# pglira/simpleICP

Measured on AMD Instinct MI355X. Metric: ICP iterations/sec (kNN correspondences/sec in `correspondences_per_s`), 10M-vs-10M pts, higher is better.
Workload: dtype f64; 1 GPU; C4 synthetic 10000000-vs-10000000 surface (SURVEY 8d generator), correspondences=1000, neighbors=10, exact 1-NN (bit-identical to brute force); n_fixed=10000000, n_movable=10000000, correspondences=1000, neighbors=10, parallelism=movable-cloud index shards x1, queries replicated

## Files before the change

### simpleicp_amd/csrc/sicp_api.cpp

```cpp
#include "sicp_host.h"
#include "../../include/simpleicp_hip_chain.h"

namespace sicph {

thread_local std::string g_err;

int fail(int code, const char *fmt, ...)
{
    char buf[512];
    va_list ap;
    va_start(ap, fmt);
    vsnprintf(buf, sizeof buf, fmt, ap);
    va_end(ap);
    g_err = buf;
    return code;
}

}

int sicp_io_fail(int code, const char *fmt, ...)
{
    char buf[512];
    va_list ap;
    va_start(ap, fmt);
// ... 154 lines not shown
    if (!ctx_out) return fail(SICP_ERR_INVALID, "ctx_out is null");
    *ctx_out = nullptr;
    int n = 0;
    if (hipGetDeviceCount(&n) != hipSuccess || n <= 0)
        return fail(SICP_ERR_NO_DEVICE, "no HIP device visible: libsimpleicp_hip has no CPU path");
    if (device < 0 || device >= n) return fail(SICP_ERR_INVALID, "device %d out of range [0,%d)", device, n);
    HIPCHK(hipSetDevice(device));
    sicp_ctx *c = new sicp_ctx();
    c->device = device;
    if (hipGetDeviceProperties(&c->prop, device) != hipSuccess) { delete c; return fail(SICP_ERR_HIP, "hipGetDeviceProperties failed"); }
    if (std::strncmp(c->prop.gcnArchName, "gfx950", 6) != 0) {
        const std::string arch = c->prop.gcnArchName;
        delete c;
        return fail(SICP_ERR_NO_DEVICE, "device %d is %s; this library carries gfx950 code only", device, arch.c_str());
    }
    if (hipStreamCreateWithFlags(&c->stream, hipStreamNonBlocking) != hipSuccess) { delete c; return fail(SICP_ERR_HIP, "hipStreamCreate failed"); }
    if (hipHostMalloc((void **)&c->h_small, H_SMALL_WORDS * sizeof(double), hipHostMallocMapped) != hipSuccess) { delete c; return fail(SICP_ERR_HIP, "hipHostMalloc failed"); }
    int rc = c->small.reserve(128);
    if (rc == SICP_OK) rc = c->ne_partial.reserve((size_t)NE_MAX_GRID * 64);
    if (rc == SICP_OK) rc = c->ticket.reserve(4);
    if (rc == SICP_OK) rc = c->icp_dev.reserve(1);
    if (rc == SICP_OK && hipStreamCreateWithFlags(&c->stream2, hipStreamNonBlocking) != hipSuccess) rc = SICP_ERR_HIP;
    if (rc == SICP_OK && hipEventCreateWithFlags(&c->pre_ev, hipEventDisableTiming) != hipSuccess) rc = SICP_ERR_HIP;
    if (rc == SICP_OK) rc = c->pre_tkt.reserve(PRE_TKT_WORDS);
    if (rc == SICP_OK && hipMemsetAsync(c->pre_tkt.p, 0, PRE_TKT_WORDS * sizeof(unsigned long long), c->stream) != hipSuccess) rc = SICP_ERR_HIP;
    if (rc == SICP_OK) rc = c->lm_dev.reserve(1);
    if (rc == SICP_OK && hipHostMalloc((void **)&c->h_lm, sizeof(LmDev), hipHostMallocDefault) != hipSuccess) rc = SICP_ERR_HIP;
    if (rc == SICP_OK) rc = c->match_work.reserve(8);
    if (rc == SICP_OK && hipMemsetAsync(c->match_work.p, 0, 8 * sizeof(unsigned long long), c->stream) != hipSuccess) rc = SICP_ERR_HIP;
    if (rc == SICP_OK && hipHostMalloc((void **)&c->h_rec, (size_t)REC_RING * REC_DOUBLES * sizeof(double), hipHostMallocMapped) != hipSuccess) rc = SICP_ERR_HIP;
    if (rc == SICP_OK && hipHostMalloc((void **)&c->h_state, sizeof(IcpDev), hipHostMallocDefault) != hipSuccess) rc = SICP_ERR_HIP;
    if (rc == SICP_OK) std::memset(c->h_rec, 0, (size_t)REC_RING * REC_DOUBLES * sizeof(double));
    if (rc == SICP_OK && hipMemsetAsync(c->ticket.p, 0, 4 * sizeof(unsigned), c->stream) != hipSuccess) rc = SICP_ERR_HIP;
    if (rc != SICP_OK) { sicp_ctx_destroy(c); return rc; }
    if (const char *e = std::getenv("SICP_ORDER_MIN_Q")) c->order_min_q = std::atol(e);
    if (const char *e = std::getenv("SICP_KNN_SWEEP")) c->knn_sweep = std::atoi(e) != 0;
    if (const char *e = std::getenv("SICP_KNN_BATCH")) c->knn_batch = std::atol(e);
    if (const char *e = std::getenv("SICP_KNN_GROUP")) c->knn_group = std::atoi(e);
    if (const char *e = std::getenv("SICP_NN16_MIN_Q")) c->nn16_min_q = std::atol(e);
    if (const char *e = std::getenv("SICP_NN16")) c->nn16_filter = !std::strcmp(e, "exact") ? 0 : !std::strcmp(e, "far") ? 1 : 2;
    if (const char *e = std::getenv("SICP_BOXES")) { c->use_boxes = std::atoi(e) != 0; c->boxes_always = std::atoi(e) >= 2; }
    if (const char *e = std::getenv("SICP_NN16F_MIN_Q")) { c->nn16f_min_q = std::atol(e); c->nn16f_min_q_forced = true; }
    if (const char *e = std::getenv("SICP_FAR_MOVE")) { const double t = std::atof(e); if (t >= 0) c->far_move = t; }
    if (const char *e = std::getenv("SICP_COARSE_MIN_N")) c->coarse_min_n = std::atol(e);
    if (const char *e = std::getenv("SICP_LM")) c->lm_one_launch = std::strcmp(e, "launches") != 0;
    if (const char *e = std::getenv("SICP_HSEL_WINDOW")) c->hsel_window = std::atoi(e) != 0;
    if (const char *e = std::getenv("SICP_TAIL_WINDOW")) c->tail_window = std::atoi(e) != 0;
    if (const char *e = std::getenv("SICP_CHAIN_PRELAUNCH")) c->chain_prelaunch = std::atoi(e) != 0;
    if (const char *e = std::getenv("SICP_TEST_BARRIER_FAULT")) c->test_barrier_fault = std::atoi(e);
    if (const char *e = std::getenv("SICP_NN_GROUP")) { const int v = std::atoi(e); if (v == 8 || v == 16) c->nn_group = v; }
    if (const char *e = std::getenv("SICP_XCHG_KEYS_MIN_Q")) c->xkeys_min_q = std::atol(e);
    if (const char *e = std::getenv("SICP_COMM_TIMEOUT_S")) { const double v = std::atof(e); if (v > 0) c->xchg_timeout_s = 2.0 * v; }
    if (const char *e = std::getenv("SICP_FSCAN")) c->fscan_variant = !std::strcmp(e, "inline") ? 1 : 0;
    if (const char *e = std::getenv("SICP_FSCAN_CAP")) c->fscan_cap = std::atol(e);
    if (const char *e = std::getenv("SICP_OUTLIER_CHUNK")) c->outlier_chunk = std::atol(e);
    if (const char *e = std::getenv("SICP_CLUSTER_CHUNK")) c->cluster_chunk = std::atol(e) > 0 ? std::atol(e) : (1L << 22);
    if (const char *e = std::getenv("SICP_FPFH_CHUNK")) c->fpfh_chunk = std::atol(e);
    if (const char *e = std::getenv("SICP_KEYPOINT_CHUNK")) c->keypoint_chunk = std::atol(e);
    if (const char *e = std::getenv("SICP_MATCH_CHUNK")) c->match_chunk = std::atol(e);
    if (const char *e = std::getenv("SICP_PLANE_SPAN")) c->plane_span = std::atol(e) > 0 ? std::atol(e) : 0;
    if (const char *e = std::getenv("SICP_ROBUST")) c->robust_path = !std::strcmp(e, "sweeps") ? 1 : !std::strcmp(e, "one") ? 2 : 0;
    if (const char *e = std::getenv("SICP_CONSISTENCY")) c->consistency_path = !std::strcmp(e, "sweeps") ? 1 : !std::strcmp(e, "one") ? 2 : 0;
    if (const char *e = std::getenv("SICP_SOLVE_TRACE")) {
        c->solve_trace = true;
        c->host_trace = std::strstr(e, "host") != nullptr;
        c->trace_sel = std::strstr(e, "sel") != nullptr; c->trace_eval = std::strstr(e, "eval") != nullptr;
    }
    if (const char *e = std::getenv("SICP_SOLVE")) c->solve_mode = !std::strcmp(e, "fused") ? 1 : !std::strcmp(e, "host") ? 2 : 0;
    if (const char *e = std::getenv("SICP_KNN1"))
        c->knn1_mode = !std::strcmp(e, "exact") ? 1 : !std::strcmp(e, "filter") ? 2 : !std::strcmp(e, "grid") ? 3 : 0;
    *ctx_out = c;
    return SICP_OK;
}

SICP_EXPORT int sicp_ctx_destroy(sicp_ctx *c)
{
    if (!c) return SICP_OK;
    (void)hipSetDevice(c->device);
    for (int s = 0; s < 2; ++s) (void)upload_join(c, s);
    if (c->copy_stream) { (void)hipStreamSynchronize(c->copy_stream); (void)hipStreamDestroy(c->copy_stream); c->copy_stream = nullptr; }
    if (c->h_bg) { (void)hipHostFree(c->h_bg); c->h_bg = nullptr; }
    c->stage_bg.release(); c->bg_small.release();
    if (c->stream) (void)hipStreamSynchronize(c->stream);
    if (c->stream2) { (void)hipStreamSynchronize(c->stream2); (void)hipStreamDestroy(c->stream2); c->stream2 = nullptr; }
    if (c->pre_ev) { (void)hipEventDestroy(c->pre_ev); c->pre_ev = nullptr; }
    c->pre_tkt.release();
    if (c->comm) { (void)rccl()->CommDestroy(c->comm); c->comm = nullptr; }
    if (c->h_dl && !c->dl_shared) (void)hipHostFree(c->h_dl);
    c->h_dl = nullptr;
    for (auto &e : c->dl_ev) if (e) { (void)hipEventDestroy(e); e = nullptr; }
    for (auto &p : c->pending) { (void)hipEventDestroy(p.a); (void)hipEventDestroy(p.b); }
    for (auto &p : c->pool) { (void)hipEventDestroy(p.a); (void)hipEventDestroy(p.b); }
    for (auto &cl : c->cloud) { cl.xyz.release(); cl.pl.release(); cl.grid.cell_start.release(); cl.grid.rec.release();
                                 cl.sub_xyz.release(); cl.sub_grid.cell_start.release(); cl.sub_grid.rec.release(); }
    c->bound_p2.release(); c->bound_d2.release(); c->bound_idx.release(); c->q_order.release(); c->k_order.release(); c->k_sel.release(); c->k_nv.release(); c->k_pl.release(); c->k_cov.release(); c->k_redo.release(); c->g_ids.release(); c->g_counts.release(); c->g_cursor.release(); c->g_blk.release(); c->match_work.release(); c->rj_keys.release();
    c->stage.release(); c->part_d2.release(); c->part_idx.release(); c->kq.release(); c->k_d2.release();
    c->k_idx.release(); c->floor_d2.release(); c->floor_idx.release(); c->bound.release(); c->hit_cnt.release(); c->hit_list.release(); c->x_send.release(); c->x_recv.release(); c->q.release(); c->normals.release();
    c->planarity.release(); c->m_idx.release(); c->m_d2.release(); c->m_p2.release(); c->dist.release();
    c->resid.release(); c->flag.release(); c->keep.release(); c->small.release(); c->ne_partial.release();
    c->lm_bar_buf.release(); c->lm_gsum.release(); c->ticket.release(); c->icp_dev.release(); c->lm_dev.release(); c->resid2.release();
    c->corr_pl.release();
    for (auto &cl : c->cloud) { cl.nv.release(); cl.nrm2.release(); cl.nrm2_have.release(); }
    c->na.cnt.release(); c->na.list_q.release(); c->na.list_m.release(); c->na.iota.release(); c->na.cov.release(); c->na.per_q.release();
    c->batch_tab.release(); c->batch_map.release();
    c->sel_blk.release(); c->sel_pos.release();
    c->vx_tab.release(); c->vx_slot.release(); c->cand_rows.release(); c->cand_keep.release(); c->cand_small.release();
    c->ev_part.release(); c->ev_out.release(); c->ev_cnt.release();
    c->ol_d.release(); c->ol_part.release(); c->ol_cnt.release();
// ... 115 lines not shown
```

### simpleicp_amd/csrc/sicp_handover.h

```cpp
#ifndef SICP_HANDOVER_H
#define SICP_HANDOVER_H

#include <cstdint>

namespace sicph {

constexpr int HANDOVER_RING = 16;

struct HandOverStep {
    int stream = 0;
    bool wait = false;
    unsigned long long wait_seq = 0;
    bool first_on_second = false;
    int slot = 0;
};

struct HandOver {
    bool road = false;
    int64_t launched = 0;
    int64_t early = 0;
    double last_seq = 0.0;
    bool second_used = false;

    HandOverStep next(double seq)
    {
        HandOverStep s;
        s.slot = (int)(launched % HANDOVER_RING);
        if (road) {
            s.stream = (int)(launched & 1);
            s.wait = launched > 0;
            s.wait_seq = s.wait ? (unsigned long long)last_seq : 0ull;
            s.first_on_second = s.stream == 1 && !second_used;
            if (s.stream == 1) second_used = true;
            if (s.wait) ++early;
        }
        last_seq = seq;
        ++launched;
        return s;
    }
};

}

#endif
```

### simpleicp_amd/csrc/sicp_host.h

```cpp
#ifndef SICP_HOST_H
#define SICP_HOST_H

#include <hip/hip_runtime.h>
#include <rccl/rccl.h>
#include <dlfcn.h>
#include <sched.h>

#include <algorithm>
#include <atomic>
#include <chrono>
#include <cmath>
#include <cstdarg>
#include <cstdio>
#include <cstdlib>
#include <cstring>
#include <limits>
#include <condition_variable>
#include <memory>
#include <mutex>
#include <string>
#include <thread>
#include <vector>

#include "../../include/simpleicp_hip.h"
// ... 86 lines not shown
    decltype(&ncclAllReduce) AllReduce = nullptr;
    decltype(&ncclGetErrorString) GetErrorString = nullptr;
    decltype(&ncclCommCount) CommCount = nullptr;
    decltype(&ncclCommUserRank) CommUserRank = nullptr;
    decltype(&ncclCommAbort) CommAbort = nullptr;
    std::string why;
};

struct NormalAngle {
    double cos_max = 0.0;
    int k = 0;
    int par = 0;
    long iota_n = 0;
    bool counters_stale = false;
    DevBuf<unsigned> cnt;
    DevBuf<uint32_t> list_q, list_m, iota;
    DevBuf<double> cov;
    DevBuf<float> per_q;
};

struct EventPair { hipEvent_t a, b; int kernel; };
constexpr int REC_RING = 16;
static_assert(REC_RING == HANDOVER_RING, "sicp_handover.h indexes the same ring");

inline long round_up(long v, long g) { return (v + g - 1) / g * g; }
inline double wall_ms() { return std::chrono::duration<double, std::milli>(std::chrono::steady_clock::now().time_since_epoch()).count(); }
inline bool is_observed(double w) { return w > 0 && std::isfinite(w); }
inline void H16_to_Xf(const double H[16], Xf *o) { for (int i = 0; i < 12; ++i) o->m[i] = H[i]; }

}
using namespace sicph;

struct BgUpload {
    std::thread th;
    bool active = false;
    int rc = SICP_OK;
    std::string err;
};

struct sicp_ctx {
    int device = 0;
    hipStream_t stream = nullptr;
    hipStream_t copy_stream = nullptr;
    BgUpload bg[2];
    DevBuf<double> stage_bg;
    DevBuf<double> bg_small;
// ... 85 lines not shown
    bool trace_sel = false, trace_eval = false;
    long solve_seq = 0;
    DevBuf<IcpDev> icp_dev;
    DevBuf<LmDev> lm_dev;
    LmDev *h_lm = nullptr;
    DevBuf<double> resid2;
    int resid_slot = 0;
    int lm_evals = 4;
    double *h_rec = nullptr;
    IcpDev *h_state = nullptr;
    DevBuf<unsigned long long> lm_bar_buf;
    unsigned long long lm_bar = 0;
    bool lm_one_launch = true;
    unsigned long long hsel_bar = 0;
    int test_barrier_fault = 0;
    bool tail_window = true;
    bool reject_prior = false;
    bool hsel_window = true;
    long hsel_run_launches = 0;
    bool hsel_dirty = false;
    int nn_group = 0;
    hipStream_t stream2 = nullptr;
    hipEvent_t pre_ev = nullptr;
    DevBuf<unsigned long long> pre_tkt;
    bool chain_prelaunch = true;
    bool pre_running = false;
    int64_t pre_last_run = 0, pre_total = 0;
    int chain_depth = 4;
    DevBuf<BatchMember> batch_tab;
    DevBuf<uint32_t> batch_map;
    double *h_batch_ring = nullptr;
    long batch_ring_members = 0;
    hipEvent_t batch_ev = nullptr;
    DevBuf<uint32_t> sel_blk;
    DevBuf<int64_t> sel_pos;
    DevBuf<int64_t> cand_rows;
    DevBuf<uint8_t> cand_keep;
    DevBuf<unsigned long long> cand_small;
    DevBuf<unsigned long long> vx_tab;
    DevBuf<uint32_t> vx_slot;
    DevBuf<double> ev_part, ev_out;
    DevBuf<long long> ev_cnt;
    DevBuf<double> ol_d, ol_part;
    DevBuf<uint32_t> ol_cnt;
    long outlier_chunk = 0;
    DevBuf<float> fp_nrm, fp_out;
    DevBuf<uint16_t> fp_cnt;
// ... 340 lines not shown
```

### simpleicp_amd/csrc/sicp_icp.cpp

```cpp
#include "sicp_host.h"
#include <map>

namespace sicph {

void euler_R(const double a[3], double R[9])
{
    const double c1 = std::cos(a[0]), s1 = std::sin(a[0]);
    const double c2 = std::cos(a[1]), s2 = std::sin(a[1]);
    const double c3 = std::cos(a[2]), s3 = std::sin(a[2]);
    R[0] = c2 * c3;                 R[1] = -c2 * s3;                R[2] = s2;
    R[3] = c1 * s3 + s1 * s2 * c3;  R[4] = c1 * c3 - s1 * s2 * s3;  R[5] = -s1 * c2;
    R[6] = s1 * s3 - c1 * s2 * c3;  R[7] = s1 * c3 + c1 * s2 * s3;  R[8] = c1 * c2;
}

void euler_dR(const double a[3], double dR[27])
{
    const double c1 = std::cos(a[0]), s1 = std::sin(a[0]);
    const double c2 = std::cos(a[1]), s2 = std::sin(a[1]);
    const double c3 = std::cos(a[2]), s3 = std::sin(a[2]);
    double *A = dR, *B = dR + 9, *C = dR + 18;
    A[0] = 0; A[1] = 0; A[2] = 0;
    A[3] = -s1 * s3 + c1 * s2 * c3;  A[4] = -s1 * c3 - c1 * s2 * s3;  A[5] = -c1 * c2;
    A[6] = c1 * s3 + s1 * s2 * c3;   A[7] = c1 * c3 - s1 * s2 * s3;   A[8] = -s1 * c2;
    B[0] = -s2 * c3;       B[1] = s2 * s3;        B[2] = c2;
// ... 171 lines not shown
    if (c->Q <= 0) return fail(SICP_ERR_INVALID, "call sicp_icp_setup first");
    CHK(check_slot(c, SICP_MOV, true));
    for (int j = 0; j < 6; ++j)
        if (std::isnan(P->obs_weight[j]) || P->obs_weight[j] < 0) return fail(SICP_ERR_INVALID, "obs_weight[%d] must be >= 0", j);
    return SICP_OK;
}

bool device_tail(const sicp_ctx *c) { return c->solve_mode != 2; }

int loop_state_init(sicp_ctx *c, const sicp_iter_params *P0)
{
    IcpDev &hs = *c->h_state;
    std::memset(&hs, 0, sizeof hs);
    double H12[12];
    params_to_H12(P0->x, H12);
    for (int j = 0; j < 6; ++j) hs.x[j] = P0->x[j];
    for (int j = 0; j < 3; ++j) { hs.sc[2 * j] = std::sin(P0->x[j]); hs.sc[2 * j + 1] = std::cos(P0->x[j]); }
    for (int i = 0; i < 12; ++i) hs.H.m[i] = H12[i];
    for (int i = 0; i < 3; ++i) {
        for (int j = 0; j < 3; ++j) hs.Hinv.m[4 * i + j] = H12[4 * j + i];
        hs.Hinv.m[4 * i + 3] = -(H12[i] * H12[3] + H12[4 + i] * H12[7] + H12[8 + i] * H12[11]);
    }
    hs.w = (P0->distance_weight > 0) ? P0->distance_weight : -1.0;
    HIPCHK(hipMemcpyAsync(c->icp_dev.p, &hs, sizeof hs, hipMemcpyHostToDevice, c->stream));
    return SICP_OK;
}

TailArgs tail_args(const sicp_ctx *c, const sicp_iter_params *P0, double min_change)
{
    const Cloud &cl = c->cloud[SICP_MOV];
    TailArgs A;
    for (int j = 0; j < 6; ++j) { A.obs[j] = P0->obs[j]; A.ow[j] = P0->obs_weight[j]; }
    A.min_change = min_change;
    A.seq = 0.0;
    A.min_planarity = (float)P0->min_planarity;
    A.max_steps = P0->max_lm_steps > 0 ? (int)P0->max_lm_steps : 100;
    A.Q = (int)c->Q;
    A.window = c->tail_window ? 1 : 0;
    A.pl2 = cl.pl_n > 0 ? cl.pl.p : nullptr;
    A.pl2_n = cl.pl_n;
    return A;
}

int take_record(sicp_ctx *c, const sicp_iter_params *P0, const double *o, sicp_iter_result *results, int64_t *done_out,
                double xcur[6], double *last_move, bool *over)
{
    const long Q = c->Q;
// ... 39 lines not shown
                             "(%lld evals %.0f, %lld steps, solves %.0f, accept %.0f) final %.0f\n",
                     o[50], o[51], o[55], o[56], o[57], o[58], o[52], o[53], (long long)R.ne_evals, o[59], (long long)R.lm_steps, o[60], o[62], o[54]);
    if (c->solve_trace && small_q && c->trace_sel)
        std::fprintf(stderr, "[sel] median: atomics+barrier %.0f fold+barrier %.0f scan+pick %.0f (more rounds %.0f) gather+barrier %.0f rank %.0f | "
                             "MAD: %.0f %.0f %.0f (%.0f) %.0f %.0f\n", o[38], o[39], o[40], o[41], o[42], o[43], o[44], o[45], o[46], o[47], o[48], o[49]);
    if (c->solve_trace && small_q && c->trace_eval)
        std::fprintf(stderr, "[eval] rows + LDS writes %.0f barrier %.0f MFMA Gram %.0f block write + barrier %.0f fold %.0f\n", o[38], o[39], o[40], o[41], o[42]);
    if (o[REC_CONVERGED] != 0.0) *over = true;
    return rc;
}


int chain_prepare(sicp_ctx *c, const sicp_iter_params *P0, bool *grid, double *last_move)
{
    c->have_corr = false;
    c->resid_sharded = false;
    *grid = takes_grid_search(c);
    if (*grid) {
        long lo0 = 0, cnt0 = c->Q;
        if (c->collective() && c->partition == SICP_PART_QUERIES) cnt0 = query_slice(c, c->Q, &lo0);
        CHK(grid_build(c, SICP_MOV, cnt0));
    }
    CHK(loop_state_init(c, P0));
    if (c->Q > SOLVE_MAX_Q) {
        const IcpDev &hs = *c->h_state;
        LmDev &hl = *c->h_lm;
        std::memset(&hl, 0, sizeof hl);
        for (int j = 0; j < 6; ++j) { hl.x[j] = hl.xt[j] = hs.x[j]; hl.sc[j] = hl.sct[j] = hs.sc[j]; }
        hl.w = hs.w; hl.first = 1;
        HIPCHK(hipMemcpyAsync(c->lm_dev.p, &hl, sizeof hl, hipMemcpyHostToDevice, c->stream));
    }
    if (normal_angle_on(c)) CHK(normal_angle_prepare(c));
    *last_move = c->have_prev_match ? c->last_move : std::numeric_limits<double>::infinity();
    return SICP_OK;
}

namespace {

struct ChainRun {
    TailArgs A;
    double seqs[REC_RING];
    double xcur[6];
    double last_move;
    int64_t launched = 0, completed = 0;
    bool grid;
    bool cold_start;
    bool over = false;
    int depth;
    int rc = SICP_OK;
    HandOver ho;
};

constexpr long PRELAUNCH_MAX_Q = 1024;

struct MatchPlan {
    bool grid = false, qshard = false;
    long lo = 0, cnt = 0;
    bool ordered = false, coarse = false, eight = false, many_q = false, boxes = false;
    bool filt = false;
    bool all_far = false;
    bool post_done = false, pack = false, pack_idx = false;
    int kernel = 0;
};

MatchPlan plan_match(const sicp_ctx *c, bool grid, int64_t iteration, bool cold_start, double last_move)
{
    const Cloud &cl = c->cloud[SICP_MOV];
    const long Q = c->Q;
    MatchPlan p;
    p.grid = grid;
    p.qshard = c->collective() && c->partition == SICP_PART_QUERIES;
    if (!grid) return p;
    p.cnt = p.qshard ? query_slice(c, Q, &p.lo) : Q;
    const long cnt = p.cnt;
// ... 1 lines not shown
    p.kernel = p.many_q ? 5 : 2;
    p.ordered = c->order_min_q > 0 && cnt >= c->order_min_q;
    p.coarse = cold_start && iteration < c->coarse_iters && cl.n >= c->coarse_min_n && cnt > 0;
    p.eight = c->nn_group ? c->nn_group == 8 : (cnt >= 196608 && !cl.grid.cap_limited && cl.grid.avg_per_cell <= 20.0);
    p.boxes = c->use_boxes && cnt > 0;
    p.filt = wants_filter(c, cl.grid, cnt);
    p.all_far = p.coarse || c->nn16_filter == 1 || cl.grid.nonuniform || !(last_move <= c->far_move * cl.grid.g.h);
    p.post_done = !c->collective() && (!p.many_q || cnt < 65536);
    p.pack = c->collective() && !p.qshard && !exchange_by_keys(c, Q);
    p.pack_idx = c->collective() && p.qshard;
    return p;
}

bool takes_prelaunch(const sicp_ctx *c, const MatchPlan &later, int64_t max_it)
{
    const Cloud &cl = c->cloud[SICP_MOV];
    return c->chain_prelaunch && c->stream2 != nullptr && max_it > 1 && c->Q <= PRELAUNCH_MAX_Q
           && (c->Q + 3) / 4 <= (long)c->prop.multiProcessorCount
           && !c->timing && !c->count_work && !c->collective() && !normal_angle_on(c) && !cl.grid.nonuniform
           && later.grid && !later.qshard && !later.many_q && !later.ordered && !later.coarse && !later.filt && later.post_done
           && !later.pack && !later.pack_idx && later.cnt == c->Q;
}

int enqueue_match(sicp_ctx *c, const TailArgs &A, const double xcur[6], MatchPlan &p, const HandOverStep *ho = nullptr)
{
    const long Q = c->Q, lo = p.lo, cnt = p.cnt;
    Cloud &cl = c->cloud[SICP_MOV];
    const double *prev = c->have_prev_match ? c->m_p2.p : nullptr;
    if (!p.grid) {
        if (p.qshard) return fail(SICP_ERR_INVALID, "query shards need the grid search (SICP_KNN1 forces another kernel)");
        double H12[12];
        params_to_H12(xcur, H12);
        Xf X; for (int i = 0; i < 12; ++i) X.m[i] = H12[i];
        return knn1_device(c, SICP_MOV, c->q.p, Q, c->qpad, &X, std::numeric_limits<double>::infinity(), prev, c->m_d2.p, c->m_idx.p,
                           c->m_p2.p);
    }
    if (p.ordered) CHK(query_order_build(c, lo, cnt, cl.grid.g.h));
    if (p.coarse) {
        CHK(subsample_build(c, SICP_MOV));
        CHK(c->bound_p2.reserve((size_t)3 * Q)); CHK(c->bound_d2.reserve(Q)); CHK(c->bound_idx.reserve(Q));
    }
    GridLevel coarse_lv; const GridLevel *coarse_grid = nullptr;
    CHK(grid_coarse_level(c, SICP_MOV, &coarse_lv, &coarse_grid));
    if (p.filt || p.boxes) CHK(grid_companions(c, cl, cl.grid, cl.n, p.filt, p.boxes));
    if (p.filt && p.coarse) CHK(grid_companions(c, cl, cl.sub_grid, cl.sub_n, true, false));
    if (p.filt && (!cl.grid.filter_ok || (p.coarse && !cl.sub_grid.filter_ok))) p.filt = false;
    GridSearch S;
    S.qx = c->q.p + lo; S.qy = c->q.p + c->qpad + lo; S.qz = c->q.p + 2 * c->qpad + lo; S.Q = cnt;
    S.order = p.ordered ? c->q_order.p : nullptr;
    set_level(S, cl.grid);
    S.coarse = coarse_grid;
    S.cell_box = p.boxes ? cl.grid.cell_box.p : nullptr;
    S.st = c->icp_dev.p;
    S.rmax = cl.rmax; S.idx_base = cl.idx_base;
    S.d2 = c->m_d2.p + lo; S.idx = c->m_idx.p + lo; S.p2 = c->m_p2.p + 3 * lo;
    S.work = c->count_work ? c->match_work.p : nullptr;
    if (p.filt) {
        const bool fill = !c->have_prev_match || c->slot_lo != lo || c->slot_cnt != cnt || c->slot_ordered != p.ordered;
        FilteredSearch F = {S, &c->q_slot, &c->p_slot, fill, nullptr, p.coarse ? &cl.sub_grid : nullptr, p.eight ? 8 : 16, p.all_far, NN_TIGHT};
        F.S.prev_p2 = S.p2;
        CHK(filtered_search(c, F));
        if (fill) { c->slot_lo = lo; c->slot_cnt = cnt; c->slot_ordered = p.ordered; }
        return SICP_OK;
    }
    Timed t(c, SICP_K_KNN1);
    if (p.coarse)
        launch_grid_nn(c->stream, bound_search(S, cl.sub_grid, c->bound_d2.p + lo, c->bound_idx.p + lo, c->bound_p2.p + 3 * lo),
                       p.many_q ? NN_LANES16 : NN_WAVE);
    if (p.pack) CHK(c->x_send.reserve((size_t)5 * Q));
// ... 85 lines not shown
    if (Q <= REJECT_MAX_Q) {
        Timed t(c, SICP_K_SELECT);
        enqueue_postmatch(c, A, post_done);
        launch_reject(c->stream, c->dist.p, c->flag.p, Q, c->keep.p, c->small.p, c->icp_dev.p, c->small.p + 4, c->tail_window && c->reject_prior);
        c->reject_prior = true;
    } else {
        enqueue_postmatch(c, A, post_done);
        Timed t(c, SICP_K_SELECT);
        CHK(reject_select(c, Q, nullptr, 0.0, c->icp_dev.p));
    }
    return enqueue_minimisation(c, A, rec);
}

int enqueue_iteration(sicp_ctx *c, ChainRun &L)
{
    const auto h0 = std::chrono::steady_clock::now();
    MatchPlan p = plan_match(c, L.grid, L.launched, L.cold_start, L.last_move);
    if (p.grid) c->last_match_kernel = p.kernel;
    if (L.ho.road) {
        L.A.seq = (double)(++c->solve_seq);
        const HandOverStep s = L.ho.next(L.A.seq);
        hipStream_t const str = s.stream ? c->stream2 : c->stream;
        if (s.first_on_second) HIPCHK(hipStreamWaitEvent(c->stream2, c->pre_ev, 0));
        CHK(enqueue_match(c, L.A, L.xcur, p, &s));
        HIPCHK(hipGetLastError());
        if (L.launched == 0) HIPCHK(hipEventRecord(c->pre_ev, c->stream));
        c->have_prev_match = true;
        L.seqs[s.slot] = L.A.seq;
        launch_icp_tail_pre(str, c->q.p, c->q.p + c->qpad, c->q.p + 2 * c->qpad, c->normals.p, c->m_p2.p, L.A, c->icp_dev.p, c->dist.p,
                            c->flag.p, c->keep.p, c->resid.p, c->h_rec + s.slot * REC_DOUBLES, c->pre_tkt.p);
        HIPCHK(hipGetLastError());
        ++L.launched;
        if (c->host_trace)
            std::fprintf(stderr, "[host] iteration %lld enqueued in %.1f us (stream %d)\n", (long long)L.launched,
                         std::chrono::duration<double, std::micro>(std::chrono::steady_clock::now() - h0).count(), s.stream);
        return SICP_OK;
    }
    CHK(enqueue_match(c, L.A, L.xcur, p));
    HIPCHK(hipGetLastError());
    c->have_prev_match = true;
    bool post_done = !p.filt && p.post_done;
    const bool packed = !p.filt && (p.pack || p.pack_idx) && p.cnt > 0;
    CHK(enqueue_exchange(c, L.A, p, packed, &post_done));
    if (normal_angle_on(c)) {
        enqueue_postmatch(c, L.A, post_done);
        post_done = true;
        CHK(normal_angle_enqueue(c, c->icp_dev.p, nullptr));
    }
    L.A.seq = (double)(++c->solve_seq);
    L.seqs[L.launched % REC_RING] = L.A.seq;
    CHK(enqueue_tail(c, L.A, post_done, c->h_rec + (L.launched % REC_RING) * REC_DOUBLES));
    HIPCHK(hipGetLastError());
    ++L.launched;
    if (c->host_trace)
        std::fprintf(stderr, "[host] iteration %lld enqueued in %.1f us\n", (long long)L.launched,
                     std::chrono::duration<double, std::micro>(std::chrono::steady_clock::now() - h0).count());
    return SICP_OK;
}

int pump_record(sicp_ctx *c, const sicp_iter_params *P0, ChainRun &L, sicp_iter_result *results, int64_t *done_out)
{
    const double *o = c->h_rec + (L.completed % REC_RING) * REC_DOUBLES;
    CHK(wait_ticket(c, o + REC_TICKET, L.seqs[L.completed % REC_RING]));
    const int status = (int)o[REC_STATUS];
    ++L.completed;
    if (status == 3) { L.over = true; return SICP_OK; }
    if (status == 4) {
        L.over = true;
        (void)hipStreamSynchronize(c->stream);
        if (L.ho.road) {
            (void)hipStreamSynchronize(c->stream2);
            HIPCHK(hipMemsetAsync(c->pre_tkt.p + PRE_ERR_WORD, 0, sizeof(unsigned long long), c->stream));
        }
        CHK(reset_barrier_state(c));
        c->have_iter = false;
        L.rc = fail(SICP_ERR_HIP, "a device-wide barrier of iteration %lld timed out (blocks not co-resident: is another process "
                                  "using the GPU?); the run was stopped and the barrier state reset", (long long)L.completed);
        return SICP_OK;
    }
    const int rr = take_record(c, P0, o, results, done_out, L.xcur, &L.last_move, &L.over);
    if (rr != SICP_OK) L.rc = rr;
    return SICP_OK;
}

}

int run_device_tail(sicp_ctx *c, const sicp_iter_params *P0, int64_t max_it, double min_change, sicp_iter_result *results,
                    int64_t *done_out)
{
    *done_out = 0;
    if (max_it <= 0) return SICP_OK;
    ChainRun L;
    CHK(chain_prepare(c, P0, &L.grid, &L.last_move));
    const bool small_q = c->Q <= SOLVE_MAX_Q;
    L.depth = !L.grid ? 1 : small_q ? c->chain_depth : std::min(c->chain_depth, 2);
    L.A = tail_args(c, P0, min_change);
    std::memcpy(L.xcur, P0->x, sizeof L.xcur);
    L.cold_start = !c->have_prev_match;
    L.ho.road = small_q && L.grid && takes_prelaunch(c, plan_match(c, L.grid, 1, L.cold_start, L.last_move), max_it);
    c->pre_last_run = 0;
    c->pre_running = L.ho.road;
    int rc = SICP_OK;
    while (true) {
        while (L.launched < max_it && L.launched - L.completed < L.depth && !L.over)
            if ((rc = enqueue_iteration(c, L)) != SICP_OK) break;
        if (rc != SICP_OK || L.completed == L.launched) break;
        if ((rc = pump_record(c, P0, L, results, done_out)) != SICP_OK) break;
    }
    c->pre_running = false;
    if (L.ho.road) {
        c->pre_last_run = L.ho.early; c->pre_total += L.ho.early;
        if (L.ho.second_used) { const hipError_t e = hipStreamSynchronize(c->stream2); if (rc == SICP_OK) HIPCHK(e); }
    }
    if (rc != SICP_OK) return rc;
    return L.rc;
}

int host_lm_solve(sicp_ctx *c, const sicp_iter_params *P, sicp_iter_result *R)
{
    const long Q = c->Q;
    int nfree = 0, freeidx[6];
    for (int j = 0; j < 6; ++j)
        if (std::isfinite(P->obs_weight[j])) freeidx[nfree++] = j;
    double *h_st = c->h_small + 160;
    double w = P->distance_weight;
    if (!(w > 0)) w = 1.0 / (R->dist_std * R->dist_std);
    R->weight_used = w;
    const double *obs = P->obs, *ow = P->obs_weight;
    double x[6]; std::memcpy(x, P->x, sizeof x);
    double ne[30];
    CHK(normal_eq_host(c, x, false, true, ne)); R->ne_evals++;
    double cost = objective(ne, w, x, obs, ow);
    double lambda = 0.0;
    const int max_steps = P->max_lm_steps > 0 ? (int)P->max_lm_steps : 100;
    for (int it = 0; it < max_steps && nfree > 0; ++it) {
// ... 353 lines not shown
```

### simpleicp_amd/csrc/sicp_internal.h

```cpp
#pragma once
#include <hip/hip_runtime.h>
#include <stdint.h>

namespace sicp {

struct Xf { double m[12]; };

constexpr int    KNN_BLOCK = 256;
constexpr int    KNN1_R    = 4;
constexpr int    TILE_PTS  = 1024;
constexpr int    FS_TILE   = 512;
constexpr int    FS_R      = 8;
constexpr int    FS_G      = 8;
constexpr int    REJECT_MAX_Q = 16384;
constexpr int    QPAD      = 2048;
constexpr int    NE_BLOCK  = 256;
constexpr int    NE_MAX_GRID = 1024;
constexpr long   STATS_MB_MIN_Q = 16384;
#define SICP_PAD_COORD 1.0e300
inline unsigned cdiv(long a, long b) { return (unsigned)((a + b - 1) / b); }

constexpr int SOLVE_MAX_Q = 2048;
void launch_fill_f32(hipStream_t s, float *dst, long n, float v);
void launch_corr_planarity(hipStream_t s, uint8_t *alive, const float *pl1, const float *pl2, float min_planarity, long Q);
// ... 170 lines not shown
                                 int64_t *idx, double *p2, double *dist, uint8_t *flag);
void launch_lexmin_gathered(hipStream_t s, const double *g, int world, long Q, double *d2, int64_t *idx, double *p2);
void launch_lexmin_postmatch(hipStream_t s, const double *g, int world, long Q, const double *qx, const double *qy, const double *qz,
                             const float *normals, const float *planarity, float min_planarity, const float *pl2, long pl2_n,
                             const IcpDev *st, double *d2, int64_t *idx, double *p2, double *dist, uint8_t *flag);
size_t reject_select_scratch_bytes();
long resident_blocks(const void *kernel, int threads);
hipError_t hsel_state_init(hipStream_t s, void *state);
hipError_t reject_by_select_one_launch(hipStream_t s, const double *dist, const uint8_t *flag, long Q, uint8_t *keep, double *out4,
                                       double *out3, void *state, unsigned long long *bar_total, double *partial, double *host_out,
                                       double seq, const IcpDev *st, unsigned absent = 0, bool use_prior = false);
void launch_aos_to_soa(hipStream_t s, const double *aos, long n, long npad, double *x, double *y, double *z);
void launch_found_mask(hipStream_t s, const int64_t *idx, long Q, uint8_t *out);
void launch_pad_fill(hipStream_t s, double *x, double *y, double *z, long n, long npad);
long eval_partials_count(long Q);
void launch_eval(hipStream_t s, const int64_t *idx, const double *d2, const double *qx, const double *qy, const double *qz, long Q,
                 double *scratch, long long *counts, double *out12);
void launch_pack_chunks(hipStream_t s, const double *x, const double *y, const double *z, long n, long CH, double *out);
void launch_soa_to_aos(hipStream_t s, const double *x, const double *y, const double *z, long n, double *aos);
void launch_transform(hipStream_t s, double *x, double *y, double *z, long n, const Xf &H);
void launch_gather_queries(hipStream_t s, const double *x, const double *y, const double *z, const int64_t *sel,
                           long Q, long qpad, double *qx, double *qy, double *qz);
void launch_aos_queries(hipStream_t s, const double *aos, long Q, long qpad, double *qx, double *qy, double *qz);
void launch_knn1_scan(hipStream_t s, const double *qx, const double *qy, const double *qz, int qpad, int qblocks,
                      const double *px, const double *py, const double *pz, long npad, int tile_step,
                      int tiles_per_chunk, int nchunks, const Xf *H, double *part_d2, uint32_t *part_idx);
void launch_knn1_fscan(hipStream_t s, int block, const double *qx, const double *qy, const double *qz, int qpad, long Q,
                       int qblocks, const double *bound, const double *px, const double *py, const double *pz,
                       int ntiles, int nparts, const Xf *H, double rmax, double *part_d2, uint32_t *part_idx);
int  fscan_blocks_per_cu(int block);
void launch_knn1_frec(hipStream_t s, int block, const double *qx, const double *qy, const double *qz, long Q, int qblocks,
                      const double *bound, const double *px, const double *py, const double *pz, int ntiles, int nparts,
                      const Xf *H, double rmax, uint32_t *hit_cnt, uint32_t *hit_list, uint32_t cap);
void launch_knn1_fixup(hipStream_t s, const double *qx, const double *qy, const double *qz, long Q, const double *px,
                       const double *py, const double *pz, const Xf *H, const uint32_t *hit_cnt, const uint32_t *hit_list,
                       uint32_t cap, uint32_t group, double max_d2, int64_t idx_base, double *d2_out, int64_t *idx_out,
                       double *p2_out, uint32_t *overflow);
int  frec_blocks_per_cu(int block);
void launch_bound_prev(hipStream_t s, const double *qx, const double *qy, const double *qz, const double *p2, long Q,
                       long qpad, const Xf &H, double *bound);
void launch_knn1_reduce(hipStream_t s, const double *part_d2, const uint32_t *part_idx, int nparts, int qpad, long Q,
                        double max_d2, int64_t idx_base, const double *px, const double *py, const double *pz,
                        double *d2_out, int64_t *idx_out, double *p2_out);
void launch_knnk_pass(hipStream_t s, int K, const double *qx, const double *qy, const double *qz, int qpad, long Q,
                      const double *px, const double *py, const double *pz, long npad, int chunk_pts, int nchunks,
                      const double *floor_d2_in, const uint32_t *floor_idx_in, double *part_d2, uint32_t *part_idx,
// ... 20 lines not shown
```

### simpleicp_amd/csrc/sicp_kernels.hip

```cpp
#include <hip/hip_runtime.h>
#include <algorithm>
#include <stdint.h>

#include "sicp_internal.h"
#include "sicp_lanes.h"
#include "sicp_normals.h"

namespace sicp {

__device__ __forceinline__ void xform(const Xf &H, double x, double y, double z,
                                      double &ox, double &oy, double &oz)
{
    double t;
    t = H.m[0] * x;  t = fma(H.m[1], y, t);  t = fma(H.m[2], z, t);   ox = t + H.m[3];
    t = H.m[4] * x;  t = fma(H.m[5], y, t);  t = fma(H.m[6], z, t);   oy = t + H.m[7];
    t = H.m[8] * x;  t = fma(H.m[9], y, t);  t = fma(H.m[10], z, t);  oz = t + H.m[11];
}

__device__ __forceinline__ double plane_dist(double dx, double dy, double dz, float nx, float ny, float nz)
{
    const double a = dx * (double)nx;
    const double b = dy * (double)ny;
    const double c = dz * (double)nz;
    return (a + b) + c;
}
// ... 30 lines not shown
    if (i >= n) return;
    const long ch = i / CH, r = i - ch * CH;
    double *o = out + 3 * ch * CH + r;
    o[0] = x[i]; o[CH] = y[i]; o[2 * CH] = z[i];
}

__global__ void k_transform(double *__restrict__ x, double *__restrict__ y, double *__restrict__ z, long n, Xf H)
{
    const long i = (long)blockIdx.x * blockDim.x + threadIdx.x;
    if (i >= n) return;
    double X, Y, Z;
    xform(H, x[i], y[i], z[i], X, Y, Z);
    x[i] = X; y[i] = Y; z[i] = Z;
}

__global__ void k_gather_queries(const double *__restrict__ x, const double *__restrict__ y,
                                 const double *__restrict__ z, const int64_t *__restrict__ sel, long Q, long qpad,
                                 double *__restrict__ qx, double *__restrict__ qy, double *__restrict__ qz)
{
    const long i = (long)blockIdx.x * blockDim.x + threadIdx.x;
    if (i >= qpad) return;
    if (i < Q) { const int64_t s = sel ? sel[i] : (int64_t)i; qx[i] = x[s]; qy[i] = y[s]; qz[i] = z[s]; }
    else       { qx[i] = 0.0; qy[i] = 0.0; qz[i] = 0.0; }
}

__global__ void k_found_mask(const int64_t *__restrict__ idx, long Q, uint8_t *__restrict__ out)
{
    const long i = (long)blockIdx.x * blockDim.x + threadIdx.x;
    if (i < Q) out[i] = idx[i] >= 0 ? 1 : 0;
}

__global__ void k_aos_queries(const double *__restrict__ aos, long Q, long qpad,
                              double *__restrict__ qx, double *__restrict__ qy, double *__restrict__ qz)
{
    const long i = (long)blockIdx.x * blockDim.x + threadIdx.x;
    if (i >= qpad) return;
    if (i < Q) { qx[i] = aos[3 * i]; qy[i] = aos[3 * i + 1]; qz[i] = aos[3 * i + 2]; }
    else       { qx[i] = 0.0; qy[i] = 0.0; qz[i] = 0.0; }
}

template <int R, bool XFORM>
__global__ __launch_bounds__(KNN_BLOCK) void k_knn1_scan(
    const double *__restrict__ qx, const double *__restrict__ qy, const double *__restrict__ qz, int qpad,
    const double *__restrict__ px, const double *__restrict__ py, const double *__restrict__ pz,
    long npad, int tile_step, int tiles_per_chunk, Xf H, double *__restrict__ part_d2,
    uint32_t *__restrict__ part_idx)
// ... 865 lines not shown
    hipLaunchKernelGGL(k_aos_to_soa, dim3(cdiv(npad, 256)), dim3(256), 0, s, aos, n, npad, x, y, z);
}
void launch_pad_fill(hipStream_t s, double *x, double *y, double *z, long n, long npad)
{
    if (npad > n) hipLaunchKernelGGL(k_pad_fill, dim3(cdiv(npad - n, 256)), dim3(256), 0, s, x, y, z, n, npad);
}
void launch_soa_to_aos(hipStream_t s, const double *x, const double *y, const double *z, long n, double *aos)
{
    if (n > 0) hipLaunchKernelGGL(k_soa_to_aos, dim3(cdiv(n, 256)), dim3(256), 0, s, x, y, z, n, aos);
}
void launch_pack_chunks(hipStream_t s, const double *x, const double *y, const double *z, long n, long CH, double *out)
{
    if (n > 0) hipLaunchKernelGGL(k_pack_chunks, dim3(cdiv(n, 256)), dim3(256), 0, s, x, y, z, n, CH, out);
}
void launch_transform(hipStream_t s, double *x, double *y, double *z, long n, const Xf &H)
{
    if (n > 0) hipLaunchKernelGGL(k_transform, dim3(cdiv(n, 256)), dim3(256), 0, s, x, y, z, n, H);
}
void launch_gather_queries(hipStream_t s, const double *x, const double *y, const double *z, const int64_t *sel,
                           long Q, long qpad, double *qx, double *qy, double *qz)
{
    hipLaunchKernelGGL(k_gather_queries, dim3(cdiv(qpad, 256)), dim3(256), 0, s, x, y, z, sel, Q, qpad, qx, qy, qz);
}
void launch_found_mask(hipStream_t s, const int64_t *idx, long Q, uint8_t *out)
{
    if (Q > 0) hipLaunchKernelGGL(k_found_mask, dim3(cdiv(Q, 256)), dim3(256), 0, s, idx, Q, out);
}
void launch_aos_queries(hipStream_t s, const double *aos, long Q, long qpad, double *qx, double *qy, double *qz)
{
    hipLaunchKernelGGL(k_aos_queries, dim3(cdiv(qpad, 256)), dim3(256), 0, s, aos, Q, qpad, qx, qy, qz);
}

void launch_knn1_scan(hipStream_t s, const double *qx, const double *qy, const double *qz, int qpad, int qblocks,
                      const double *px, const double *py, const double *pz, long npad, int tile_step,
                      int tiles_per_chunk, int nchunks, const Xf *H, double *part_d2, uint32_t *part_idx)
{
    const dim3 grid(qblocks, nchunks), block(KNN_BLOCK);
    Xf id = {};
    if (H)
        hipLaunchKernelGGL((k_knn1_scan<KNN1_R, true>), grid, block, 0, s, qx, qy, qz, qpad, px, py, pz, npad,
                           tile_step, tiles_per_chunk, *H, part_d2, part_idx);
    else
        hipLaunchKernelGGL((k_knn1_scan<KNN1_R, false>), grid, block, 0, s, qx, qy, qz, qpad, px, py, pz, npad,
                           tile_step, tiles_per_chunk, id, part_d2, part_idx);
}

// ... 191 lines not shown
```

Before: 57140 iterations/s.

## Pass loop state by kernel argument, hoist match setup, end chain on device

The initial ICP loop state (and the LM state for large Q) is now written by a tiny kernel that carries the state image as a kernel argument, instead of host-to-device memcpys from pinned memory. Match preparation (query ordering, subsampling, grid companions) is hoisted ahead of the first launch so the second stream's event is recorded earlier. The run also ends by ordering the main stream behind stream2 with an event rather than a host stream synchronize. The aim is to cut host-side latency and stalls at the start and end of each chained run, at the cost of more control flags and an extra event.

```diff
diff --git a/simpleicp_amd/csrc/sicp_api.cpp b/simpleicp_amd/csrc/sicp_api.cpp
--- a/simpleicp_amd/csrc/sicp_api.cpp
+++ b/simpleicp_amd/csrc/sicp_api.cpp
@@ -200,6 +200,7 @@
     if (rc == SICP_OK) rc = c->icp_dev.reserve(1);
     if (rc == SICP_OK && hipStreamCreateWithFlags(&c->stream2, hipStreamNonBlocking) != hipSuccess) rc = SICP_ERR_HIP;
     if (rc == SICP_OK && hipEventCreateWithFlags(&c->pre_ev, hipEventDisableTiming) != hipSuccess) rc = SICP_ERR_HIP;
+    if (rc == SICP_OK && hipEventCreateWithFlags(&c->end_ev, hipEventDisableTiming) != hipSuccess) rc = SICP_ERR_HIP;
     if (rc == SICP_OK) rc = c->pre_tkt.reserve(PRE_TKT_WORDS);
     if (rc == SICP_OK && hipMemsetAsync(c->pre_tkt.p, 0, PRE_TKT_WORDS * sizeof(unsigned long long), c->stream) != hipSuccess) rc = SICP_ERR_HIP;
     if (rc == SICP_OK) rc = c->lm_dev.reserve(1);
@@ -225,6 +226,7 @@
     if (const char *e = std::getenv("SICP_HSEL_WINDOW")) c->hsel_window = std::atoi(e) != 0;
     if (const char *e = std::getenv("SICP_TAIL_WINDOW")) c->tail_window = std::atoi(e) != 0;
     if (const char *e = std::getenv("SICP_CHAIN_PRELAUNCH")) c->chain_prelaunch = std::atoi(e) != 0;
+    if (const char *e = std::getenv("SICP_RUN_ENTRY")) c->run_entry = std::atoi(e) & 7;
     if (const char *e = std::getenv("SICP_TEST_BARRIER_FAULT")) c->test_barrier_fault = std::atoi(e);
     if (const char *e = std::getenv("SICP_NN_GROUP")) { const int v = std::atoi(e); if (v == 8 || v == 16) c->nn_group = v; }
     if (const char *e = std::getenv("SICP_XCHG_KEYS_MIN_Q")) c->xkeys_min_q = std::atol(e);
@@ -262,6 +264,7 @@
     if (c->stream) (void)hipStreamSynchronize(c->stream);
     if (c->stream2) { (void)hipStreamSynchronize(c->stream2); (void)hipStreamDestroy(c->stream2); c->stream2 = nullptr; }
     if (c->pre_ev) { (void)hipEventDestroy(c->pre_ev); c->pre_ev = nullptr; }
+    if (c->end_ev) { (void)hipEventDestroy(c->end_ev); c->end_ev = nullptr; }
     c->pre_tkt.release();
     if (c->comm) { (void)rccl()->CommDestroy(c->comm); c->comm = nullptr; }
     if (c->h_dl && !c->dl_shared) (void)hipHostFree(c->h_dl);
diff --git a/simpleicp_amd/csrc/sicp_handover.h b/simpleicp_amd/csrc/sicp_handover.h
--- a/simpleicp_amd/csrc/sicp_handover.h
+++ b/simpleicp_amd/csrc/sicp_handover.h
@@ -12,11 +12,21 @@
     bool wait = false;
     unsigned long long wait_seq = 0;
     bool first_on_second = false;
+    bool setup_before = false;
+    bool setup_after = false;
     int slot = 0;
+};
+
+enum HandOverEnd {
+    HANDOVER_END_NONE = 0,
+    HANDOVER_END_DEVICE = 1,
+    HANDOVER_END_HOST = 2
 };
 
 struct HandOver {
     bool road = false;
+    bool setup_ahead = true;
+    bool device_end = true;
     int64_t launched = 0;
     int64_t early = 0;
     double last_seq = 0.0;
@@ -33,10 +43,18 @@
             s.first_on_second = s.stream == 1 && !second_used;
             if (s.stream == 1) second_used = true;
             if (s.wait) ++early;
+            s.setup_before = launched == 0 && setup_ahead;
+            s.setup_after = launched == 0 && !setup_ahead;
         }
         last_seq = seq;
         ++launched;
         return s;
+    }
+
+    HandOverEnd end(bool ok) const
+    {
+        if (!road || !second_used) return HANDOVER_END_NONE;
+        return ok && device_end ? HANDOVER_END_DEVICE : HANDOVER_END_HOST;
     }
 };
 
diff --git a/simpleicp_amd/csrc/sicp_host.h b/simpleicp_amd/csrc/sicp_host.h
--- a/simpleicp_amd/csrc/sicp_host.h
+++ b/simpleicp_amd/csrc/sicp_host.h
@@ -132,6 +132,9 @@
 struct EventPair { hipEvent_t a, b; int kernel; };
 constexpr int REC_RING = 16;
 static_assert(REC_RING == HANDOVER_RING, "sicp_handover.h indexes the same ring");
+constexpr int RUN_ENTRY_STATE_BY_ARG = 1;
+constexpr int RUN_ENTRY_SETUP_AHEAD = 2;
+constexpr int RUN_ENTRY_DEVICE_END = 4;
 
 inline long round_up(long v, long g) { return (v + g - 1) / g * g; }
 inline double wall_ms() { return std::chrono::duration<double, std::milli>(std::chrono::steady_clock::now().time_since_epoch()).count(); }
@@ -263,7 +266,9 @@
     int nn_group = 0;
     hipStream_t stream2 = nullptr;
     hipEvent_t pre_ev = nullptr;
+    hipEvent_t end_ev = nullptr;
     DevBuf<unsigned long long> pre_tkt;
+    int run_entry = RUN_ENTRY_STATE_BY_ARG | RUN_ENTRY_SETUP_AHEAD | RUN_ENTRY_DEVICE_END;
     bool chain_prelaunch = true;
     bool pre_running = false;
     int64_t pre_last_run = 0, pre_total = 0;
diff --git a/simpleicp_amd/csrc/sicp_icp.cpp b/simpleicp_amd/csrc/sicp_icp.cpp
--- a/simpleicp_amd/csrc/sicp_icp.cpp
+++ b/simpleicp_amd/csrc/sicp_icp.cpp
@@ -217,7 +217,19 @@
         hs.Hinv.m[4 * i + 3] = -(H12[i] * H12[3] + H12[4 + i] * H12[7] + H12[8 + i] * H12[11]);
     }
     hs.w = (P0->distance_weight > 0) ? P0->distance_weight : -1.0;
+    LmDev *hl = c->Q > SOLVE_MAX_Q ? c->h_lm : nullptr;
+    if (hl) {
+        std::memset(hl, 0, sizeof *hl);
+        for (int j = 0; j < 6; ++j) { hl->x[j] = hl->xt[j] = hs.x[j]; hl->sc[j] = hl->sct[j] = hs.sc[j]; }
+        hl->w = hs.w; hl->first = 1;
+    }
+    if (c->run_entry & RUN_ENTRY_STATE_BY_ARG) {
+        launch_state_store(c->stream, hs, c->icp_dev.p, hl, c->lm_dev.p);
+        HIPCHK(hipGetLastError());
+        return SICP_OK;
+    }
     HIPCHK(hipMemcpyAsync(c->icp_dev.p, &hs, sizeof hs, hipMemcpyHostToDevice, c->stream));
+    if (hl) HIPCHK(hipMemcpyAsync(c->lm_dev.p, hl, sizeof *hl, hipMemcpyHostToDevice, c->stream));
     return SICP_OK;
 }
 
@@ -303,14 +315,6 @@
         CHK(grid_build(c, SICP_MOV, cnt0));
     }
     CHK(loop_state_init(c, P0));
-    if (c->Q > SOLVE_MAX_Q) {
-        const IcpDev &hs = *c->h_state;
-        LmDev &hl = *c->h_lm;
-        std::memset(&hl, 0, sizeof hl);
-        for (int j = 0; j < 6; ++j) { hl.x[j] = hl.xt[j] = hs.x[j]; hl.sc[j] = hl.sct[j] = hs.sc[j]; }
-        hl.w = hs.w; hl.first = 1;
-        HIPCHK(hipMemcpyAsync(c->lm_dev.p, &hl, sizeof hl, hipMemcpyHostToDevice, c->stream));
-    }
     if (normal_angle_on(c)) CHK(normal_angle_prepare(c));
     *last_move = c->have_prev_match ? c->last_move : std::numeric_limits<double>::infinity();
     return SICP_OK;
@@ -330,7 +334,14 @@
     int depth;
     int rc = SICP_OK;
     HandOver ho;
+    std::chrono::steady_clock::time_point t0;
 };
+
+void trace_stamp(const sicp_ctx *c, const ChainRun &L, const char *what)
+{
+    if (!c->host_trace) return;
+    std::fprintf(stderr, "[host] +%.1f us %s\n", std::chrono::duration<double, std::micro>(std::chrono::steady_clock::now() - L.t0).count(), what);
+}
 
 constexpr long PRELAUNCH_MAX_Q = 1024;
 
@@ -378,6 +389,22 @@
            && !later.pack && !later.pack_idx && later.cnt == c->Q;
 }
 
+int match_prepare(sicp_ctx *c, MatchPlan &p, GridLevel *coarse_lv, const GridLevel **coarse_grid)
+{
+    const long Q = c->Q;
+    Cloud &cl = c->cloud[SICP_MOV];
+    if (p.ordered) CHK(query_order_build(c, p.lo, p.cnt, cl.grid.g.h));
+    if (p.coarse) {
+        CHK(subsample_build(c, SICP_MOV));
+        CHK(c->bound_p2.reserve((size_t)3 * Q)); CHK(c->bound_d2.reserve(Q)); CHK(c->bound_idx.reserve(Q));
+    }
+    CHK(grid_coarse_level(c, SICP_MOV, coarse_lv, coarse_grid));
+    if (p.filt || p.boxes) CHK(grid_companions(c, cl, cl.grid, cl.n, p.filt, p.boxes));
+    if (p.filt && p.coarse) CHK(grid_companions(c, cl, cl.sub_grid, cl.sub_n, true, false));
+    if (p.filt && (!cl.grid.filter_ok || (p.coarse && !cl.sub_grid.filter_ok))) p.filt = false;
+    return SICP_OK;
+}
+
 int enqueue_match(sicp_ctx *c, const TailArgs &A, const double xcur[6], MatchPlan &p, const HandOverStep *ho = nullptr)
 {
     const long Q = c->Q, lo = p.lo, cnt = p.cnt;
@@ -391,16 +418,8 @@
         return knn1_device(c, SICP_MOV, c->q.p, Q, c->qpad, &X, std::numeric_limits<double>::infinity(), prev, c->m_d2.p, c->m_idx.p,
                            c->m_p2.p);
     }
-    if (p.ordered) CHK(query_order_build(c, lo, cnt, cl.grid.g.h));
-    if (p.coarse) {
-        CHK(subsample_build(c, SICP_MOV));
-        CHK(c->bound_p2.reserve((size_t)3 * Q)); CHK(c->bound_d2.reserve(Q)); CHK(c->bound_idx.reserve(Q));
-    }
     GridLevel coarse_lv; const GridLevel *coarse_grid = nullptr;
-    CHK(grid_coarse_level(c, SICP_MOV, &coarse_lv, &coarse_grid));
-    if (p.filt || p.boxes) CHK(grid_companions(c, cl, cl.grid, cl.n, p.filt, p.boxes));
-    if (p.filt && p.coarse) CHK(grid_companions(c, cl, cl.sub_grid, cl.sub_n, true, false));
-    if (p.filt && (!cl.grid.filter_ok || (p.coarse && !cl.sub_grid.filter_ok))) p.filt = false;
+    CHK(match_prepare(c, p, &coarse_lv, &coarse_grid));
     GridSearch S;
     S.qx = c->q.p + lo; S.qy = c->q.p + c->qpad + lo; S.qz = c->q.p + 2 * c->qpad + lo; S.Q = cnt;
     S.order = p.ordered ? c->q_order.p : nullptr;
@@ -532,9 +551,14 @@
         const HandOverStep s = L.ho.next(L.A.seq);
         hipStream_t const str = s.stream ? c->stream2 : c->stream;
         if (s.first_on_second) HIPCHK(hipStreamWaitEvent(c->stream2, c->pre_ev, 0));
+        if (s.setup_before) {
+            GridLevel lv; const GridLevel *lvp = nullptr;
+            CHK(match_prepare(c, p, &lv, &lvp));
+            HIPCHK(hipEventRecord(c->pre_ev, c->stream));
+        }
         CHK(enqueue_match(c, L.A, L.xcur, p, &s));
         HIPCHK(hipGetLastError());
-        if (L.launched == 0) HIPCHK(hipEventRecord(c->pre_ev, c->stream));
+        if (s.setup_after) HIPCHK(hipEventRecord(c->pre_ev, c->stream));
         c->have_prev_match = true;
         L.seqs[s.slot] = L.A.seq;
         launch_icp_tail_pre(str, c->q.p, c->q.p + c->qpad, c->q.p + 2 * c->qpad, c->normals.p, c->m_p2.p, L.A, c->icp_dev.p, c->dist.p,
@@ -544,6 +568,7 @@
         if (c->host_trace)
             std::fprintf(stderr, "[host] iteration %lld enqueued in %.1f us (stream %d)\n", (long long)L.launched,
                          std::chrono::duration<double, std::micro>(std::chrono::steady_clock::now() - h0).count(), s.stream);
+        trace_stamp(c, L, "enqueue_iteration returns");
         return SICP_OK;
     }
     CHK(enqueue_match(c, L.A, L.xcur, p));
@@ -565,6 +590,7 @@
     if (c->host_trace)
         std::fprintf(stderr, "[host] iteration %lld enqueued in %.1f us\n", (long long)L.launched,
                      std::chrono::duration<double, std::micro>(std::chrono::steady_clock::now() - h0).count());
+    trace_stamp(c, L, "enqueue_iteration returns");
     return SICP_OK;
 }
 
@@ -601,13 +627,18 @@
     *done_out = 0;
     if (max_it <= 0) return SICP_OK;
     ChainRun L;
+    L.t0 = std::chrono::steady_clock::now();
+    trace_stamp(c, L, "run_device_tail entered");
     CHK(chain_prepare(c, P0, &L.grid, &L.last_move));
+    trace_stamp(c, L, "chain_prepare returned");
     const bool small_q = c->Q <= SOLVE_MAX_Q;
     L.depth = !L.grid ? 1 : small_q ? c->chain_depth : std::min(c->chain_depth, 2);
     L.A = tail_args(c, P0, min_change);
     std::memcpy(L.xcur, P0->x, sizeof L.xcur);
     L.cold_start = !c->have_prev_match;
     L.ho.road = small_q && L.grid && takes_prelaunch(c, plan_match(c, L.grid, 1, L.cold_start, L.last_move), max_it);
+    L.ho.setup_ahead = (c->run_entry & RUN_ENTRY_SETUP_AHEAD) != 0;
+    L.ho.device_end = (c->run_entry & RUN_ENTRY_DEVICE_END) != 0;
     c->pre_last_run = 0;
     c->pre_running = L.ho.road;
     int rc = SICP_OK;
@@ -618,9 +649,18 @@
         if ((rc = pump_record(c, P0, L, results, done_out)) != SICP_OK) break;
     }
     c->pre_running = false;
+    trace_stamp(c, L, "last pump_record returned");
     if (L.ho.road) {
         c->pre_last_run = L.ho.early; c->pre_total += L.ho.early;
-        if (L.ho.second_used) { const hipError_t e = hipStreamSynchronize(c->stream2); if (rc == SICP_OK) HIPCHK(e); }
+        switch (L.ho.end(rc == SICP_OK && L.rc == SICP_OK)) {
+        case HANDOVER_END_DEVICE:
+            HIPCHK(hipEventRecord(c->end_ev, c->stream2));
+            HIPCHK(hipStreamWaitEvent(c->stream, c->end_ev, 0));
+            break;
+        case HANDOVER_END_HOST: { const hipError_t e = hipStreamSynchronize(c->stream2); if (rc == SICP_OK) HIPCHK(e); break; }
+        case HANDOVER_END_NONE: break;
+        }
+        trace_stamp(c, L, "second stream ordered behind");
     }
     if (rc != SICP_OK) return rc;
     return L.rc;
diff --git a/simpleicp_amd/csrc/sicp_internal.h b/simpleicp_amd/csrc/sicp_internal.h
--- a/simpleicp_amd/csrc/sicp_internal.h
+++ b/simpleicp_amd/csrc/sicp_internal.h
@@ -216,6 +216,7 @@
 void launch_gather_queries(hipStream_t s, const double *x, const double *y, const double *z, const int64_t *sel,
                            long Q, long qpad, double *qx, double *qy, double *qz);
 void launch_aos_queries(hipStream_t s, const double *aos, long Q, long qpad, double *qx, double *qy, double *qz);
+void launch_state_store(hipStream_t s, const IcpDev &hs, IcpDev *st, const LmDev *hl, LmDev *lm);
 void launch_knn1_scan(hipStream_t s, const double *qx, const double *qy, const double *qz, int qpad, int qblocks,
                       const double *px, const double *py, const double *pz, long npad, int tile_step,
                       int tiles_per_chunk, int nchunks, const Xf *H, double *part_d2, uint32_t *part_idx);
diff --git a/simpleicp_amd/csrc/sicp_kernels.hip b/simpleicp_amd/csrc/sicp_kernels.hip
--- a/simpleicp_amd/csrc/sicp_kernels.hip
+++ b/simpleicp_amd/csrc/sicp_kernels.hip
@@ -1,6 +1,7 @@
 #include <hip/hip_runtime.h>
 #include <algorithm>
 #include <stdint.h>
+#include <string.h>
 
 #include "sicp_internal.h"
 #include "sicp_lanes.h"
@@ -77,6 +78,24 @@
     if (i >= qpad) return;
     if (i < Q) { const int64_t s = sel ? sel[i] : (int64_t)i; qx[i] = x[s]; qy[i] = y[s]; qz[i] = z[s]; }
     else       { qx[i] = 0.0; qy[i] = 0.0; qz[i] = 0.0; }
+}
+
+constexpr int ST_WORDS = sizeof(IcpDev) / 8, LM_WORDS = sizeof(LmDev) / 8;
+static_assert(sizeof(IcpDev) == 344 && sizeof(IcpDev) % 8 == 0 && ST_WORDS <= 64, "the loop state leaves k_state_store as one 64-lane store");
+static_assert(sizeof(LmDev) % 8 == 0 && sizeof(IcpDev) + sizeof(LmDev) + 16 <= 4096, "both images fit a kernel's argument segment");
+struct StateImage { unsigned long long w[ST_WORDS]; };
+struct LmImage { unsigned long long w[LM_WORDS]; };
+__global__ __launch_bounds__(64) void k_state_store(unsigned long long *__restrict__ st, StateImage img)
+{
+    const int l = threadIdx.x;
+    if (l < ST_WORDS) st[l] = img.w[l];
+}
+__global__ __launch_bounds__(64) void k_state_store_lm(unsigned long long *__restrict__ st, unsigned long long *__restrict__ lm,
+                                                       StateImage img, LmImage lmg)
+{
+    const int l = threadIdx.x;
+    if (l < ST_WORDS) st[l] = img.w[l];
+    for (int i = l; i < LM_WORDS; i += 64) lm[i] = lmg.w[i];
 }
 
 __global__ void k_found_mask(const int64_t *__restrict__ idx, long Q, uint8_t *__restrict__ out)
@@ -988,6 +1007,15 @@
 {
     hipLaunchKernelGGL(k_gather_queries, dim3(cdiv(qpad, 256)), dim3(256), 0, s, x, y, z, sel, Q, qpad, qx, qy, qz);
 }
+void launch_state_store(hipStream_t s, const IcpDev &hs, IcpDev *st, const LmDev *hl, LmDev *lm)
+{
+    StateImage img;
+    memcpy(img.w, &hs, sizeof hs);
+    if (!hl) { hipLaunchKernelGGL(k_state_store, dim3(1), dim3(64), 0, s, (unsigned long long *)st, img); return; }
+    LmImage lmg;
+    memcpy(lmg.w, hl, sizeof *hl);
+    hipLaunchKernelGGL(k_state_store_lm, dim3(1), dim3(64), 0, s, (unsigned long long *)st, (unsigned long long *)lm, img, lmg);
+}
 void launch_found_mask(hipStream_t s, const int64_t *idx, long Q, uint8_t *out)
 {
     if (Q > 0) hipLaunchKernelGGL(k_found_mask, dim3(cdiv(Q, 256)), dim3(256), 0, s, idx, Q, out);
```

Result: no change. 56610 iterations/s (-0.9%).
